# GalDude33/Fetal-MRI-Segmentation

Hardware: AMD Instinct MI355X
Metric: 3D patches/sec (64x128x128, bf16) fwd+bwd (higher is better)
Workload: dtype bf16

## Files before the change

### fetal-mri-segmentation_amd/csrc/conv3d_api.hip

```cpp
#include "common.h"

int conv3d_fwd_generic(const void*, int, int, int, const void*, int, const void*, const float*, const void*, void*, int, int, int, int, int,
                       int, float, int, hipStream_t);
int conv3d_wgrad_generic(const void*, int, int, int, const void*, int, const void*, float*, float*, int, int, int, int, int, int,
                         hipStream_t);
bool conv3d_fwd_mfma_ok(int C0, int C1, int Cout, int D, int H, int W, int dtype);
bool conv3d_wgrad_mfma_ok(int C0, int C1, int Cout, int D, int H, int W, int dtype);
bool conv3d_fwd_needs_cube(int D, int H, int W);
bool conv3d_wgrad_cout32_ok(int C0, int C1, int Cout, int N, int D, int H, int W, int dtype, int planar, int up0);
int conv3d_fwd_mfma(const void*, int, int, int, const void*, int, const void*, const float*, const void*, void*, int, int, int, int, int, int,
                    float, int, hipStream_t);
int conv3d_wgrad_mfma_f32(const void*, int, int, const void*, int, const void*, float*, float*, int, int, int, int, int, hipStream_t);
int conv3d_wgrad_mfma(const void*, int, int, int, const void*, int, const void*, float*, float*, int, int, int, int, int, void*, int64_t,
                      hipStream_t);
int64_t conv3d_wgrad_mfma_ws_bytes(int C0, int C1, int Cout, int N, int D, int H, int W, int planar);
int conv3d_upcat_wgrad_mfma(const void*, int, const void*, int, const void*, float*, float*, float*, int, int, int, int, int, int, void*, int64_t,
                            hipStream_t);
int conv3d_fwd_mfma_ex(int, const void*, int, int, int, const void*, int, const void*, const float*, const void*, const void*, void*, int, int, int,
                       int, int, int, float, int, hipStream_t);

int conv3d_upcat_wgrad_mfma_ex(const void*, int, const void*, int, const void*, float*, float*, float*, int, int, int, int, int, int, int, void*,
                               int64_t, hipStream_t);
int conv3d_fwd_mfma_res_b27(const void*, int, const void*, const float*, const void*, void*, int, int, int, int, int, int, float, int, hipStream_t);
int conv3d_fwd_tail_ok(int C0, int Cout, int N, int D, int H, int W, int dtype, int planar);
int conv3d_fwd_mfma_tail(const void*, int, const void*, const float*, void*, void*, const float*, const float*, float*, int, int, int, int, int, int,
                         float, int, int, hipStream_t);

int conv3d_fwd_ntail_ok(int C0, int C1, int Cout, int N, int D, int H, int W, int dtype);
int conv3d_fwd_mfma_ntail(int, const void*, int, int, const void*, int, const void*, const float*, const void*, void*, int, int, int, int, int, int,
                          float, double*, int, const float*, hipStream_t);
int norm_ws_zero(double* ws, int n, hipStream_t s);
int norm_ws_fold(double* ws, int nslot, int n, hipStream_t s);
int conv3d_fwd_ntail_slots();

bool conv3d_first_ok(int C0, int C1, int Cout, int D, int H, int W, int dtype, int up0, int planar);
int conv3d_first_fwd(const void*, int, int, const void*, const float*, void*, int, int, int, int, int, int, float, hipStream_t);
int conv3d_first_wgrad(const void*, int, int, const void*, float*, float*, int, int, int, int, int, hipStream_t);
bool conv3d_first_dgrad_ok(int Cin, int Cout, int D, int H, int W, int dtype);
int conv3d_first_dgrad(const void*, int, const void*, float*, int, int, int, int, int, hipStream_t);

static int check_common(const void* src0, int C0, int up0, int planar, const void* src1, int C1, int N, int D, int H, int W, int Cout) {
    if (N <= 0 || D <= 0 || H <= 0 || W <= 0 || Cout <= 0 || C0 <= 0 || C1 < 0) return FMRI_E_SHAPE;
    if (!src0 || (C1 > 0 && !src1)) return FMRI_E_SHAPE;
// ... 287 lines not shown
                if (!(cd == 1 && ch == 1 && cw == 1) && acc[ch][cw] != 0.f) atomicAdd(&out[((cd * 3 + ch) * 3 + cw) * C + c], acc[ch][cw]);
    }
}
}
extern "C" int fmri_conv3d_upcat_fwd_bias27(const void* src0_low, int C0, const void* src1, int C1, const void* w_up_fwd, const void* w_skip_fwd,
                                            const float* bias27, void* y, int N, int D, int H, int W, int Cout, int act, float alpha, int dtype,
                                            fmri_stream_t stream) {
    if (!src0_low || !src1 || !w_up_fwd || !w_skip_fwd || !bias27 || !y || N <= 0 || C1 <= 0) return FMRI_E_SHAPE;
    if (!(upcat_ok(C0, C1, Cout, D, H, W, dtype, 0) & 1)) return FMRI_E_SHAPE;
    if ((((uintptr_t)src0_low) | ((uintptr_t)src1) | ((uintptr_t)w_up_fwd) | ((uintptr_t)w_skip_fwd) | ((uintptr_t)y) | ((uintptr_t)bias27)) & 15) return FMRI_E_ALIGN;
    int rc = conv3d_fwd_mfma_ex(1, src0_low, C0, 0, 0, nullptr, 0, w_up_fwd, nullptr, nullptr, nullptr, y, N, D / 2, H / 2, W / 2, Cout, FMRI_ACT_NONE, 0.f,
                                dtype, as_stream(stream));
    if (rc) return rc;
    return conv3d_fwd_mfma_res_b27(src1, C1, w_skip_fwd, bias27, y, y, N, D, H, W, Cout, act, alpha, dtype, as_stream(stream));
}
extern "C" int fmri_conv3d_upcat_wgrad_parts(const void* src0_low, int C0, const void* src1, int C1, const void* dy, float* dw, float* db,
                                             float* dwc, int N, int D, int H, int W, int Cout, int dtype, void* workspace, int64_t workspace_bytes,
                                             fmri_stream_t stream) {
    if (!src0_low || !dy || !dw || !dwc || N <= 0 || C1 <= 0 || !src1) return FMRI_E_SHAPE;
    if (!(upcat_ok(C0, C1, Cout, D, H, W, dtype, 0) & 2)) return FMRI_E_SHAPE;
    if ((((uintptr_t)src0_low) | ((uintptr_t)src1) | ((uintptr_t)dy)) & 15) return FMRI_E_ALIGN;
    return conv3d_upcat_wgrad_mfma_ex(src0_low, C0, src1, C1, dy, dw, db, dwc, N, D, H, W, Cout, 0, 0, workspace, workspace_bytes, as_stream(stream));
}
extern "C" int fmri_border_class_sums(const void* dy, float* out27, int N, int D, int H, int W, int C, int dtype, fmri_stream_t stream) {
    if (!dy || !out27 || N <= 0 || D < 2 || H < 2 || W < 2 || C <= 0) return FMRI_E_SHAPE;
    hipStream_t s = as_stream(stream);
    const dim3 grid(N * D, H >= 64 ? 8 : (H >= 16 ? 4 : 1));
    if (dtype == FMRI_BF16) k_border_class_sums<bf16_t><<<grid, 256, 0, s>>>((const bf16_t*)dy, out27, D, H, W, C);
    else if (dtype == FMRI_F32) k_border_class_sums<float><<<grid, 256, 0, s>>>((const float*)dy, out27, D, H, W, C);
    else return FMRI_E_DTYPE;
    FMRI_LAUNCH_CHECK();
    return FMRI_OK;
}

extern "C" int64_t fmri_norm_tail_ws_doubles(int G, int C) { return (int64_t)(1 + conv3d_fwd_ntail_slots()) * G * C * 2; }
extern "C" int fmri_conv3d_fwd_ntail_ok(int C0, int C1, int Cout, int N, int D, int H, int W, int dtype) {
    if (N <= 0 || D <= 0 || H <= 0 || W <= 0 || C0 <= 0 || C1 < 0 || Cout <= 0) return 0;
    return conv3d_fwd_ntail_ok(C0, C1, Cout, N, D, H, W, dtype);
}
extern "C" int fmri_conv3d_fwd_stats(const void* src0, int C0, int up0, const void* src1, int C1, const void* w, const float* bias, void* y,
                                     int N, int D, int H, int W, int Cout, int act, float alpha, double* ws, int per_instance, int dtype,
                                     fmri_stream_t stream) {
    int rc = check_common(src0, C0, up0, 0, src1, C1, N, D, H, W, Cout);
    if (rc) return rc;
    if (!ws || !w || !y || !conv3d_fwd_ntail_ok(C0, C1, Cout, N, D, H, W, dtype)) return FMRI_E_SHAPE;
    if ((((uintptr_t)src0) | ((uintptr_t)src1) | ((uintptr_t)w) | ((uintptr_t)y) | ((uintptr_t)ws)) & 15) return FMRI_E_ALIGN;
// ... 85 lines not shown
```

### fetal-mri-segmentation_amd/csrc/conv3d_wgrad.hip

```cpp
#define FMRI_MFMA_TU_WGRAD
#include "mfma_common.h"

FMRI_DET_TU(mfma)

namespace {

namespace wg {
constexpr int TH = 8, TW = 16;
constexpr int XH = TH + 2, XW = TW + 2;
constexpr int XROWS = XH * XW;
constexpr int YROWS = TH * TW;
constexpr int NTHREADS = 256;
}


template <int ROWB> __device__ __forceinline__ int wg_slot_off(int row, int slot) {
    if (ROWB == 128) return row * 128 + ((slot ^ (((row >> 1) & 1) << 2)) << 4);
    return row * 64 + (slot << 4);
}

template <int ROWB>
__device__ __forceinline__ bf16x8_t tr_frag(const unsigned char* base, int row0, int tile32, int lane) {
    const int g = lane >> 4, q = (lane & 15) >> 2, p = lane & 3, hk = g >> 1;
    const int rowa = row0 + 8 * hk + q, rowb = rowa + 4;
// ... 567 lines not shown
__global__ void __launch_bounds__(256, F32 ? 1 : 2) k_conv_wgrad_kd(WkArgs a) {
    __shared__ __attribute__((aligned(16))) unsigned char lds[WkCfg<F32>::LDS_BYTES];
    const int lane = threadIdx.x & 63;
    const int wv = __builtin_amdgcn_readfirstlane(threadIdx.x >> 6);
    switch (wv & 3) {
        case 0: wk_run<0, F32>(a, lds, wv, lane); break;
        case 1: wk_run<1, F32>(a, lds, wv, lane); break;
        case 2: wk_run<2, F32>(a, lds, wv, lane); break;
        default: wk_run<3, F32>(a, lds, wv, lane); break;
    }
}

struct WuCfg {
    static constexpr int NW = 4;
    static constexpr int ROWB = 128, RS = 8;
    static constexpr int X_INSTR = (wg::XROWS * RS + 63) / 64;
    static constexpr int Y_INSTR = wg::YROWS * RS / 64;
    static constexpr int XS_BYTES = X_INSTR * 1024, YS_BYTES = Y_INSTR * 1024;
    static constexpr int NXS = 3, NYS = 2;
    static constexpr int LDS_BYTES = NXS * XS_BYTES + NYS * YS_BYTES;
    static constexpr int XPW = (X_INSTR + NW - 1) / NW, YPW = Y_INSTR / NW;
    static constexpr int PF = 3;
    static constexpr int SP0 = 1, SPD = 2;
};

template <int G>
__device__ __forceinline__ void wu_run(const WkArgs& a, unsigned char* lds, int wv, int lane) {
    typedef WuCfg K;
    constexpr int KDP = G >> 1, KHP = G & 1, NW = K::NW, ROWB = K::ROWB, RS = K::RS;
    constexpr int NI = 2;
    constexpr int XPW = K::XPW, YPW = K::YPW;
    typedef __attribute__((ext_vector_type(8))) short s16x8;
    const SrcB& s = a.s;
    const int N = a.N, D = a.D, H = a.H, W = a.W, Cout = a.Cout;
    const int Cin = s.C0;
    const int ncib = Cin / 64, ncob = Cout / 64;
    const int ncombo = 8 * ncob * ncib;
    const int wg_id = xcd_logical_id(blockIdx.x, gridDim.x);
    int combo = wg_id % ncombo;
    const int slab = wg_id / ncombo;
    const int cib = combo % ncib; combo /= ncib;
    const int cob = combo % ncob;
    const int par = combo / ncob;
    const int pd = par >> 2, ph = (par >> 1) & 1, pw = par & 1;
    const int co0 = cob * 64, cc = cib * 64;
    const int r = lane & 31, hk = lane >> 5;
    const bool do_bias = G == 0 && a.db != nullptr && cib == 0;

    f32x16 acc[2][2][NI];
#pragma unroll
    for (int q = 0; q < 4 * NI; ++q)
#pragma unroll
        for (int k = 0; k < 16; ++k) acc[q / (2 * NI)][(q / NI) & 1][q % NI][k] = 0.f;
    float bsum[2] = {0.f, 0.f};

    const int twn = W / wg::TW, thn = H / wg::TH;
    const int nunits = N * D * thn * twn;
    const unsigned lds0 = __builtin_amdgcn_readfirstlane(lds_addr(lds));

    int cn = 0, ch0 = 0, cw0 = 0;
    int x_off[XPW], y_off[YPW];
    unsigned x_ok = 0;
    auto col_setup = [&](int n, int h0, int w0) {
        cn = n; ch0 = h0; cw0 = w0;
        x_ok = 0;
#pragma unroll
        for (int k = 0; k < XPW; ++k) {
            const int id = wv + NW * k;
            const int i = id * 64 + lane;
            const int row = i / RS, ps = i % RS;
            const int ls = ps ^ (((row >> 1) & 1) << 2);
            const int xh = row / wg::XW, xw = row % wg::XW;
            const int gh = h0 - 1 + xh, gw = w0 - 1 + xw;
            const bool ok = id < K::X_INSTR && row < wg::XROWS && (unsigned)gh < (unsigned)H && (unsigned)gw < (unsigned)W;
            const int ghc = min(max(gh, 0), H - 1), gwc = min(max(gw, 0), W - 1);
            x_off[k] = ((ghc * W + gwc) * Cin + ls * 8) * 2;
// ... 1 lines not shown
        }
#pragma unroll
        for (int k = 0; k < YPW; ++k) {
            const int id = (NW - 1 - wv) + NW * k;
            const int i = id * 64 + lane;
            const int row = i / RS, ps = i % RS;
            const int ls = ps ^ (((row >> 1) & 1) << 2);
            y_off[k] = (((row >> 4) * 4 * W + (row & 15) * 2) * Cout + ls * 8) * 2;
        }
    };
    auto x_rsrc = [&](int gd) {
        const bool dok = (unsigned)gd < (unsigned)D;
        const int gdc = min(max(gd, 0), D - 1);
        return dma_rsrc(s.p0 + ((int64_t)cn * D + gdc) * H * W * Cin + cc, dok ? (int)DMA_OOB : 0);
    };
    auto y_rsrc = [&](int d) {
        return dma_rsrc(a.dy + ((((int64_t)cn * 2 * D + 2 * d + pd) * 2 * H + 2 * ch0 + ph) * 2 * W + 2 * cw0 + pw) * Cout + co0);
    };
    auto x_piece = [&](i32x4 rs, int slot, int k) {
        const int id = wv + NW * k;
        if (id < K::X_INSTR)
            dma16_buf(rs, ((x_ok >> k) & 1) ? (unsigned)x_off[k] : DMA_OOB, __builtin_amdgcn_readfirstlane(lds0 + slot * K::XS_BYTES + id * 1024));
    };
    auto y_piece = [&](i32x4 rs, int ybuf, int k) {
        const int id = (NW - 1 - wv) + NW * k;
        dma16_buf(rs, (unsigned)y_off[k], __builtin_amdgcn_readfirstlane(lds0 + K::NXS * K::XS_BYTES + ybuf * K::YS_BYTES + id * 1024));
    };
    auto issue_x = [&](int gd, int slot) {
        const i32x4 rs = x_rsrc(gd);
#pragma unroll
        for (int k = 0; k < XPW; ++k) x_piece(rs, slot, k);
    };
    auto issue_y = [&](int d, int ybuf) {
        const i32x4 rs = y_rsrc(d);
#pragma unroll
        for (int k = 0; k < YPW; ++k) y_piece(rs, ybuf, k);
    };

    const int gq = lane >> 4, qd = (lane & 15) >> 2, pp = lane & 3;
    const int lrow = 8 * (gq >> 1) + qd;
    const int lslot = 2 * (gq & 1) + (pp >> 1);
    const int shift = ph * wg::XW + pw;
    int pre_x[4];
#pragma unroll
    for (int m = 0; m < 4; ++m) pre_x[m] = wg_slot_off<ROWB>(lrow + shift + m, lslot) + (pp & 1) * 8;
    const int pre_y = wg_slot_off<ROWB>(lrow, lslot) + (pp & 1) * 8;

    const int per = (nunits + a.nslab - 1) / a.nslab;
    int u = slab * per;
    const int u_end = min(nunits, u + per);
    if (u < u_end) {
        int d;
        {
            int q = u;
            d = q % D; q /= D;
            const int w0 = (q % twn) * wg::TW; q /= twn;
            col_setup(q / thn, (q % thn) * wg::TH, w0);
        }
        issue_x(d + pd - 1, 0);
// ... 2 lines not shown
        int lo = 0, yb = 0;
#ifdef FMRI_PROF
        unsigned long long wprof[12] = {};
        PROF_T(wk0);
#endif
        for (; u < u_end; ++u) {
            PROF_T(w0);
            asm volatile("s_waitcnt vmcnt(0)" ::: "memory");
            PROF_T(w1);
            __builtin_amdgcn_s_barrier();
            PROF_T(w2);
            const bool more = u + 1 < u_end;
            const bool fresh = more && d + 1 == D;
            if (more && fresh) {
                int w0 = cw0 + wg::TW, h0 = ch0, n = cn;
                if (w0 == W) { w0 = 0; h0 += wg::TH; if (h0 == H) { h0 = 0; ++n; } }
                col_setup(n, h0, w0);
                d = -1;
            }
            PROF_T(w3);
            const int hi = lo == 2 ? 0 : lo + 1, fr = hi == 2 ? 0 : hi + 1;
            int xbase = (KDP ? hi : lo) * K::XS_BYTES;
            asm volatile("" : "+s"(xbase));
            const int ybase = K::NXS * K::XS_BYTES + yb * K::YS_BYTES;
            const int nyb = yb ^ 1;
            i32x4 nx_rs = {0, 0, 0, 0}, ny_rs = {0, 0, 0, 0};
            auto load_a = [&](int ks8, s16x8 (&av)[2]) {
#pragma unroll
                for (int h = 0; h < 2; ++h) {
                    const unsigned char* p0 = lds + ybase + (h ? (pre_y ^ 64) : pre_y) + ks8 * wg::TW * ROWB;
                    s16x4 v0 = __builtin_amdgcn_ds_read_tr16_b64_v4i16((lds_s16x4*)p0);
                    s16x4 v1 = __builtin_amdgcn_ds_read_tr16_b64_v4i16((lds_s16x4*)(p0 + 4 * ROWB));
                    av[h] = __builtin_shufflevector(v0, v1, 0, 1, 2, 3, 4, 5, 6, 7);
                }
            };
            auto load_b = [&](int st) {
                const int ks8 = st / (2 * NI), j = (st / NI) & 1, i = st % NI;
                const int c = (ks8 + KHP) * wg::XW + j;
                const unsigned char* pb = lds + xbase + (i ? (pre_x[c & 3] ^ 64) : pre_x[c & 3]) + (c >> 2) * 4 * ROWB;
                s16x4 v0 = __builtin_amdgcn_ds_read_tr16_b64_v4i16((lds_s16x4*)pb);
                s16x4 v1 = __builtin_amdgcn_ds_read_tr16_b64_v4i16((lds_s16x4*)(pb + 4 * ROWB));
                return __builtin_shufflevector(v0, v1, 0, 1, 2, 3, 4, 5, 6, 7);
            };
            constexpr int NS = 16 * NI, PF = K::PF, RING = PF + 1;
            s16x8 av[2][2], b[RING];
#pragma unroll
            for (int q = 0; q < PF; ++q) b[q] = load_b(q);
            load_a(0, av[0]);
#pragma unroll
            for (int st = 0; st < NS; ++st) {
                const int ks8 = st / (2 * NI), j = (st / NI) & 1, i = st % NI, ab = ks8 & 1;
                if (st + PF < NS) b[(st + PF) % RING] = load_b(st + PF);
                if (st % (2 * NI) == 1 && ks8 + 1 < 8) load_a(ks8 + 1, av[ab ^ 1]);
                if (st % (2 * NI) == 0 && do_bias) {
#pragma unroll
                    for (int h = 0; h < 2; ++h)
#pragma unroll
                        for (int q = 0; q < 8; ++q) bsum[h] += bf2f((unsigned short)av[ab][h][q]);
                }
                const bf16x8_t bb = __builtin_bit_cast(bf16x8_t, b[st % RING]);
#pragma unroll
                for (int h = 0; h < 2; ++h)
                    acc[j][h][i] = __builtin_amdgcn_mfma_f32_32x32x16_bf16(__builtin_bit_cast(bf16x8_t, av[ab][h]), bb, acc[j][h][i], 0, 0, 0);
                if (more) {
                    if (st == 0) {
                        nx_rs = x_rsrc(fresh ? pd - 1 : d + 1 + pd);
                        ny_rs = y_rsrc(d + 1);
                    }
                    if (st >= K::SP0 && (st - K::SP0) % K::SPD == 0 && (st - K::SP0) / K::SPD < XPW + YPW) {
                        const int pc = (st - K::SP0) / K::SPD;
                        if (pc < YPW) y_piece(ny_rs, nyb, pc);
                        else x_piece(nx_rs, fr, pc - YPW);
                    }
                }
                __builtin_amdgcn_sched_barrier(0);
            }
            asm volatile("s_waitcnt lgkmcnt(0)" ::: "memory");
            PROF_T(w4);
#ifdef FMRI_PROF
            wprof[0] += w1 - w0; wprof[1] += w2 - w1; wprof[2] += w3 - w2; wprof[3] += w4 - w3; wprof[6] += 1;
#endif
            if (fresh) {
                __builtin_amdgcn_s_barrier();
                issue_x(pd, lo);
                lo = fr;
            } else {
                lo = hi;
            }
            yb ^= 1;
            ++d;
#ifdef FMRI_PROF
            { PROF_T(w5); wprof[4] += w5 - w4; }
#endif
        }
#ifdef FMRI_PROF
        { PROF_T(wk1); wprof[5] = wk1 - wk0; }
        if (lane == 0) for (int i = 0; i < 7; ++i) atomicAdd(&g_prof[i], wprof[i]);
#endif
    }
#pragma unroll
    for (int j = 0; j < 2; ++j)
#pragma unroll
        for (int h = 0; h < 2; ++h)
#pragma unroll
            for (int i = 0; i < NI; ++i)
#pragma unroll
                for (int reg = 0; reg < 16; ++reg) {
                    const int co = co0 + h * 32 + (reg & 3) + 8 * (reg >> 2) + 4 * hk;
                    const int ci = cc + i * 32 + r;
                    atomicAdd(&a.dw[((int64_t)((par * 2 + KDP) * 4 + KHP * 2 + j) * Cout + co) * Cin + ci], acc[j][h][i][reg]);
                }
    if (do_bias) {
#pragma unroll
        for (int h = 0; h < 2; ++h) {
            float bq = bsum[h];
            bq += __shfl_down(bq, 32);
            if (hk == 0) atomicAdd(&a.db[co0 + h * 32 + r], bq);
        }
    }
}

__global__ void __launch_bounds__(256, 1) k_conv_wgrad_up_kd(WkArgs a) {
    __shared__ __attribute__((aligned(16))) unsigned char lds[WuCfg::LDS_BYTES];
    const int lane = threadIdx.x & 63;
    const int wv = __builtin_amdgcn_readfirstlane(threadIdx.x >> 6);
    switch (wv & 3) {
        case 0: wu_run<0>(a, lds, wv, lane); break;
        case 1: wu_run<1>(a, lds, wv, lane); break;
        case 2: wu_run<2>(a, lds, wv, lane); break;
        default: wu_run<3>(a, lds, wv, lane); break;
    }
}

template <int CIB>
__global__ void __launch_bounds__(256)
k_wgrad_reduce(const float* __restrict__ ws, float* __restrict__ dw, int Cout, int Cin, int nslab, int ncombo, int ncob, int ncib,
               int planar, int ksp) {
    constexpr int PER4 = 9 * 64 * CIB / 4;
    __shared__ float4 red[8][32];
    const int tx = threadIdx.x & 31, ty = threadIdx.x >> 5;
    const int64_t col = (int64_t)blockIdx.x * 32 + tx;
    const bool ok = col < (int64_t)ncombo * PER4;
    float4 a0 = make_float4(0.f, 0.f, 0.f, 0.f), a1 = a0, a2 = a0, a3 = a0;
    int combo = 0, e4 = 0;
    if (ok) {
        combo = (int)(col / PER4);
        e4 = (int)(col % PER4);
        const int nsl = nslab * ksp;
        const float4* base = reinterpret_cast<const float4*>(ws) + e4;
        int j = ty;
        for (; j + 24 < nsl; j += 32) {
            const int64_t i0 = ((int64_t)(j / ksp) * ncombo + combo) * ksp + (j % ksp);
            const int64_t i1 = ((int64_t)((j + 8) / ksp) * ncombo + combo) * ksp + ((j + 8) % ksp);
// ... 145 lines not shown
        const int64_t q = i / C0;
        const int co = (int)(q % Cout);
        const int t = (int)(q / Cout) + (planar ? 9 : 0);
        const int kd = t / 9, kh = (t / 3) % 3, kw = t % 3;
        float acc = 0.f;
        if (planar) {
#pragma unroll
            for (int p = 0; p < 4; ++p) {
                const int cls = tap_class_w(p >> 1, kh) * 2 + tap_class_w(p & 1, kw);
                acc += dwc[((int64_t)(p * 4 + cls) * Cout + co) * C0 + c0];
            }
        } else {
#pragma unroll
            for (int p = 0; p < 8; ++p) {
                const int cls = (tap_class_w(p >> 2, kd) * 2 + tap_class_w((p >> 1) & 1, kh)) * 2 + tap_class_w(p & 1, kw);
                acc += dwc[((int64_t)(p * 8 + cls) * Cout + co) * C0 + c0];
            }
        }
        dw[((int64_t)t * Cout + co) * dw_ld + c0] += acc;
    }
}
}

int conv3d_upcat_wgrad_mfma_ex(const void* src0_low, int C0, const void* src1, int C1, const void* dy, float* dw, float* db, float* dwc, int N,
                               int D, int H, int W, int Cout, int planar, int expand, void* workspace, int64_t workspace_bytes, hipStream_t st);
int conv3d_upcat_wgrad_mfma(const void* src0_low, int C0, const void* src1, int C1, const void* dy, float* dw, float* db, float* dwc, int N,
                            int D, int H, int W, int Cout, int planar, void* workspace, int64_t workspace_bytes, hipStream_t st) {
    return conv3d_upcat_wgrad_mfma_ex(src0_low, C0, src1, C1, dy, dw, db, dwc, N, D, H, W, Cout, planar, 1, workspace, workspace_bytes, st);
}
int conv3d_upcat_wgrad_mfma_ex(const void* src0_low, int C0, const void* src1, int C1, const void* dy, float* dw, float* db, float* dwc, int N,
                               int D, int H, int W, int Cout, int planar, int expand, void* workspace, int64_t workspace_bytes, hipStream_t st) {
    if (hipMemsetAsync(dwc, 0, (size_t)(planar ? 16 : 64) * Cout * C0 * sizeof(float), st) != hipSuccess) return FMRI_E_LAUNCH;
    {
        SrcB s{(const bf16_t*)src0_low, nullptr, C0, 0, 0, planar ? 0 : 1, planar};
        const int Dl = planar ? D : D / 2, Hl = H / 2, Wl = W / 2;
        const bool wide = C0 % 64 == 0;
        const int CIB = wide ? 64 : 32;
        const int combos = (planar ? 4 : 16) * (Cout / 64) * (C0 / CIB);
        const int nunits = N * Dl * (Hl / wg::TH) * (Wl / wg::TW);
        int nslab = (1536 + combos - 1) / combos;
        if (nslab > nunits) nslab = nunits;
        if (nslab < 1) nslab = 1;
        float* const dbu = C1 == 0 ? db : nullptr;
        static const int upw_kd = env_int("FMRI_UPW_KD", 1, {0, 1});
        if (upw_kd && !planar && wide && Cout % 64 == 0) {
            const int combos_kd = 8 * (Cout / 64) * (C0 / 64);
            int nsl = (fwd_cu_count() + combos_kd - 1) / combos_kd;
            if (nsl > nunits) nsl = nunits;
            if (nsl < 1) nsl = 1;
            const WkArgs wa{s, (const bf16_t*)dy, dwc, dbu, N, Dl, Hl, Wl, Cout, nsl, C0};
            k_conv_wgrad_up_kd<<<combos_kd * nsl, 256, 0, st>>>(wa);
        } else if (wide) k_conv_wgrad_mfma<2, true><<<combos * nslab, wg::NTHREADS, 0, st>>>(s, (const bf16_t*)dy, dwc, dbu, N, Dl, Hl, Wl, Cout, nslab, nullptr, C0);
        else k_conv_wgrad_mfma<1, true><<<combos * nslab, wg::NTHREADS, 0, st>>>(s, (const bf16_t*)dy, dwc, dbu, N, Dl, Hl, Wl, Cout, nslab, nullptr, C0);
    }
    if (expand) k_expand_up_wgrad<<<grid_for((int64_t)(planar ? 9 : 27) * Cout * C0, 256, 1024), 256, 0, st>>>(dwc, dw, Cout, C0, C0 + C1, planar);
    FMRI_LAUNCH_CHECK();
    if (C1 == 0) return FMRI_OK;
    return conv3d_wgrad_mfma_ld(src1, C1, 0, planar, nullptr, 0, dy, dw + C0, C0 + C1, db, N, D, H, W, Cout, workspace, workspace_bytes, st);
}
```

### fetal-mri-segmentation_amd/fmri_hip/_lib.py

```python
import ctypes as C
import os

F32, BF16 = 0, 1
F64 = 3
ACT_NONE, ACT_RELU, ACT_LEAKY = 0, 1, 2
IMPL_AUTO, IMPL_GENERIC, IMPL_MFMA = 0, 1, 2

_HERE = os.path.dirname(os.path.abspath(__file__))
LIB_PATH = os.environ.get("FMRI_LIB") or os.path.join(os.path.dirname(_HERE), "lib", "libfmri_hip.so")


class LibraryMissing(RuntimeError):
    pass


class FmriError(RuntimeError):
    pass


p, i32, i64, f32 = C.c_void_p, C.c_int, C.c_int64, C.c_float
u64, u32 = C.c_uint64, C.c_uint32

SIGNATURES = {
    "fmri_version": [],
# ... 82 lines not shown
    "fmri_rmsprop_step": [p, p, p, i64, f32, f32, f32, f32, p, f32, f32, p],
    "fmri_adam_step_ex": [p, p, p, p, p, i64, f32, f32, f32, f32, f32, p, f32, f32, p],
    "fmri_set_deterministic": [p, p, i64],
    "fmri_deterministic_finish": [p, p, i64, p],
    "fmri_set_deterministic_scratch": [p, i64],
    "fmri_norm_det_workspace_bytes": [i32, i64, i32, i32],
    "fmri_tile_gather": [p, i32, i32, i32, p, i32, i32, i32, i32, p, i32, p],
    "fmri_tile_gather_stack": [p, p, i32, i32, i32, p, i32, i32, i32, i32, i32, i32, p, i32, p],
    "fmri_tile_scatter_accumulate": [p, p, i32, i32, i32, i32, i32, p, p, i32, i32, i32, p],
    "fmri_tile_finalize": [p, p, p, p, i64, i32, p],
    "fmri_volume_pad_flip": [p, i32, i32, i32, i32, p, i32, i32, i32, i32, p, i32, C.c_double, p],
    "fmri_tile_finalize_flip": [p, p, i32, i32, i32, i32, p, i32, i32, i32, p, i32, p, p],
    "fmri_labels_expand_u8": [p, i64, p, i32, p, p],
    "fmri_tile_finalize_labels": [p, p, p, p, i64, i32, C.c_double, p, p],
    "fmri_cast": [p, i32, p, i32, i64, p],
    "fmri_conv3d_upcat_ok": [i32, i32, i32, i32, i32, i32, i32],
    "fmri_conv3d_upcat_fwd_bias27": [p, i32, p, i32, p, p, p, p, i32, i32, i32, i32, i32, i32, f32, i32, p],
    "fmri_conv3d_upcat_wgrad_parts": [p, i32, p, i32, p, p, p, p, i32, i32, i32, i32, i32, i32, p, i64, p],
    "fmri_border_class_sums": [p, p, i32, i32, i32, i32, i32, i32, p],
    "fmri_conv3d_pack_up_weights": [p, i32, i32, i32, p, p, p, p, i32, p],
    "fmri_conv3d_upcat_fwd": [p, i32, p, i32, p, p, p, p, i32, i32, i32, i32, i32, i32, f32, i32, p],
    "fmri_conv3d_upcat_dgrad": [p, i32, p, p, p, p, p, p, i32, i32, i32, i32, i32, i32, i32, p],
    "fmri_conv3d_stride2_fwd": [p, i32, p, p, p, i32, i32, i32, i32, i32, i32, p],
    "fmri_conv3d_upcat_wgrad": [p, i32, p, i32, p, p, p, p, i32, i32, i32, i32, i32, i32, p, i64, p],
    "fmri_conv2d_upcat_ok": [i32, i32, i32, i32, i32, i32, i32],
    "fmri_conv2d_pack_up_weights": [p, i32, i32, i32, p, p, p, p, i32, p],
    "fmri_conv2d_upcat_fwd": [p, i32, p, i32, p, p, p, p, i32, i32, i32, i32, i32, f32, i32, p],
    "fmri_conv2d_upcat_dgrad": [p, i32, p, p, p, p, p, p, i32, i32, i32, i32, i32, i32, p],
    "fmri_conv2d_upcat_wgrad": [p, i32, p, i32, p, p, p, p, i32, i32, i32, i32, i32, p, i64, p],
    "fmri_sigmoid_dice_fwd_weighted": [p, p, p, p, p, i64, p],
    "fmri_sigmoid_loss_bwd_weighted": [p, p, p, p, p, i64, i32, f32, f32, f32, p],
    "fmri_minmax": [p, i64, i32, p, p],
    "fmri_rescale_intensity": [p, i64, i32, p, i32, f32, f32, f32, p],
    "fmri_noise_augment": [p, i64, i32, p, p, i32, f32, p],
    "fmri_shot_noise_step": [p, i64, i32, p, p, p, p, i32, p],
    "fmri_correlate1d_f32": [p, p, i32, i32, i32, i32, p, i32, i32, p],
    "fmri_coarse_dropout": [p, i32, i32, i32, i32, i32, p, i32, i32, i32, p, p],
    "fmri_minmax_ws_batch": [p, i64, i64, i32, i32, p, p, p],
    "fmri_rescale_intensity_ws_batch": [p, i64, i64, i32, i32, p, p, p, p],
    "fmri_affine_sample_batch": [i32, p, p, p, p, i32, i32, p, p, i32, i32, i32, i32, i32, p, i32, i32, i64, p],
    "fmri_mri_intensity_ws_batch": [p, i32, i32, i32, i64, i32, i32, p, p, p, p, p],
    "fmri_noise_rng_batch": [p, i64, i64, i32, i32, p, p, i32, f32, u64, p, p],
    "fmri_shot_noise_rng_batch": [p, i64, i64, i32, i32, p, p, u64, p, p],
    "fmri_elastic_fields_rng_batch": [p, i32, i32, i32, p, p, u64, p, i32, p],
    "fmri_elastic_warp_batch": [p, i32, i32, i32, i32, i32, i64, p, i32, p, i32, i64, i32, p],
    "fmri_coarse_dropout_rng_batch": [p, i32, i32, i32, i32, i32, i64, i32, p, i32, f32, p, u64, p, p],
# ... 36 lines not shown
```

### fetal-mri-segmentation_amd/fmri_hip/ops.py

```python
import torch

from ._lib import lib, check, F32, BF16, F64, ACT_NONE, ACT_RELU, IMPL_AUTO


def dt(t):
    if t.dtype == torch.float32:
        return F32
    if t.dtype == torch.bfloat16:
        return BF16
    raise TypeError("unsupported dtype %s" % t.dtype)


import os as _os

_raw_stream = getattr(torch._C, "_cuda_getCurrentRawStream", None) if _os.environ.get("FMRI_RAW_STREAM", "1") != "0" else None
_cur_device = getattr(torch._C, "_cuda_getDevice", None)


def _s():
    if _raw_stream is not None and _cur_device is not None:
        return _raw_stream(_cur_device())
    return torch.cuda.current_stream().cuda_stream


# ... 695 lines not shown
    _need_cuda(x, w_s2_fwd, bias, y)
    N, D, H, W, Cin = x.shape
    Cout = y.shape[-1]
    assert tuple(y.shape) == (N, D // 2, H // 2, W // 2, Cout) and tuple(w_s2_fwd.shape) == (8, 8, Cout, Cin)
    assert bias is None or (bias.dtype == torch.float32 and bias.numel() >= Cout)
    check(lib().fmri_conv3d_stride2_fwd(_p(x), Cin, _p(w_s2_fwd), _p(bias), _p(y), N, D, H, W, Cout, dt(x), _s()), "fmri_conv3d_stride2_fwd")
    return y


def conv3d_upcat_wgrad(src0_low, src1, dy, dw, db, dwc_scratch, workspace=None, planar=False):
    _need_cuda(src0_low, src1, dy, dw, db, dwc_scratch, workspace)
    N, D, H, W, Cout = dy.shape
    C0, C1 = src0_low.shape[-1], (0 if src1 is None else src1.shape[-1])
    assert dwc_scratch.dtype == torch.float32 and dwc_scratch.numel() >= (16 if planar else 64) * Cout * C0
    nws = 0 if workspace is None else workspace.numel() * workspace.element_size()
    if planar:
        assert N == 1
        check(lib().fmri_conv2d_upcat_wgrad(_p(src0_low), C0, _p(src1), C1, _p(dy), _p(dw), _p(db), _p(dwc_scratch), D, H, W, Cout, dt(dy),
                                            _p(workspace), nws, _s()), "fmri_conv2d_upcat_wgrad")
        return
    check(lib().fmri_conv3d_upcat_wgrad(_p(src0_low), C0, _p(src1), C1, _p(dy), _p(dw), _p(db), _p(dwc_scratch), N, D, H, W, Cout, dt(dy),
                                        _p(workspace), nws, _s()),
          "fmri_conv3d_upcat_wgrad")


def conv3d_upcat_fwd_bias27(src0_low, src1, w_up_f, w_sk_f, bias27, y, act=ACT_RELU, alpha=0.0):
    _need_cuda(src0_low, src1, w_up_f, w_sk_f, bias27, y)
    N, D, H, W, Cout = y.shape
    assert bias27.dtype == torch.float32 and tuple(bias27.shape) == (27, Cout) and bias27.is_contiguous()
    check(lib().fmri_conv3d_upcat_fwd_bias27(_p(src0_low), src0_low.shape[-1], _p(src1), src1.shape[-1], _p(w_up_f), _p(w_sk_f), _p(bias27), _p(y),
                                             N, D, H, W, Cout, act, float(alpha), dt(y), _s()), "fmri_conv3d_upcat_fwd_bias27")
    return y


def conv3d_upcat_wgrad_parts(src0_low, src1, dy, dw, db, dwc, workspace=None):
    _need_cuda(src0_low, src1, dy, dw, db, dwc, workspace)
    N, D, H, W, Cout = dy.shape
    C0, C1 = src0_low.shape[-1], src1.shape[-1]
    assert dwc.dtype == torch.float32 and dwc.numel() >= 64 * Cout * C0 and tuple(dw.shape) == (27, Cout, C0 + C1)
    nws = 0 if workspace is None else workspace.numel() * workspace.element_size()
    check(lib().fmri_conv3d_upcat_wgrad_parts(_p(src0_low), C0, _p(src1), C1, _p(dy), _p(dw), _p(db), _p(dwc), N, D, H, W, Cout, dt(dy), _p(workspace),
                                              nws, _s()), "fmri_conv3d_upcat_wgrad_parts")


def border_class_sums(dy, out27):
    _need_cuda(dy, out27)
# ... 951 lines not shown
```

### include/fmri_hip.h

```cpp
#ifndef FMRI_HIP_H
#define FMRI_HIP_H
#include <stddef.h>
#include <stdint.h>

#ifdef __cplusplus
extern "C" {
#endif

typedef void* fmri_stream_t;

enum { FMRI_OK = 0, FMRI_E_SHAPE = -1, FMRI_E_ALIGN = -2, FMRI_E_ARCH = -3, FMRI_E_LAUNCH = -4, FMRI_E_DTYPE = -5 };
enum { FMRI_F32 = 0, FMRI_BF16 = 1, FMRI_U8 = 2 ,
       FMRI_F64 = 3  };
enum { FMRI_ACT_NONE = 0, FMRI_ACT_RELU = 1, FMRI_ACT_LEAKY = 2 };
enum { FMRI_IMPL_AUTO = 0, FMRI_IMPL_GENERIC = 1, FMRI_IMPL_MFMA = 2 };

int fmri_version(void);
const char* fmri_error_string(int code);
int fmri_clock_stamp(unsigned long long* out16, fmri_stream_t stream);
int fmri_conv3d_uses_mfma(int C0, int C1, int Cout, int D, int H, int W, int dtype);

int fmri_conv3d_fwd(const void* src0, int C0, int up0, const void* src1, int C1, const void* w, const float* bias,
                    const void* mask, void* y, int N, int D, int H, int W, int Cout, int act, float alpha, int dtype,
                    int impl, int planar, fmri_stream_t stream);
// ... 23 lines not shown
int fmri_conv3d_upcat_fwd_bias27(const void* src0_low, int C0, const void* src1, int C1, const void* w_up_fwd, const void* w_skip_fwd,
                                 const float* bias27, void* y, int N, int D, int H, int W, int Cout, int act, float alpha, int dtype,
                                 fmri_stream_t stream);
int fmri_conv3d_upcat_wgrad_parts(const void* src0_low, int C0, const void* src1, int C1, const void* dy, float* dw, float* db, float* dwc,
                                  int N, int D, int H, int W, int Cout, int dtype, void* workspace, int64_t workspace_bytes,
                                  fmri_stream_t stream);
int fmri_border_class_sums(const void* dy, float* out27, int N, int D, int H, int W, int C, int dtype, fmri_stream_t stream);

int fmri_conv3d_upcat_ok(int C0, int C1, int Cout, int D, int H, int W, int dtype);
int fmri_conv3d_pack_up_weights(const float* w, int C0, int C1, int Cout, void* w_up_fwd, void* w_up_dgrad, void* w_skip_fwd,
                                void* w_skip_dgrad, int dtype, fmri_stream_t stream);
int fmri_conv3d_upcat_fwd(const void* src0_low, int C0, const void* src1, int C1, const void* w_up_fwd, const void* w_skip_fwd,
                          const float* bias, void* y, int N, int D, int H, int W, int Cout, int act, float alpha, int dtype,
                          fmri_stream_t stream);
int fmri_conv3d_upcat_dgrad(const void* dy, int Cout, const void* w_up_dgrad, const void* w_skip_dgrad, const void* mask_low,
                            const void* mask_skip, void* dx_low, void* dx_skip, int N, int D, int H, int W, int C0, int C1, int dtype,
                            fmri_stream_t stream);
int fmri_conv3d_stride2_fwd(const void* x, int Cin, const void* w_s2_fwd, const float* bias, void* y, int N, int D, int H, int W, int Cout, int dtype,
                            fmri_stream_t stream);

int fmri_conv3d_upcat_wgrad(const void* src0_low, int C0, const void* src1, int C1, const void* dy, float* dw, float* db,
                            float* dwc_scratch, int N, int D, int H, int W, int Cout, int dtype, void* workspace, int64_t workspace_bytes,
                            fmri_stream_t stream);

int fmri_conv2d_upcat_ok(int C0, int C1, int Cout, int S, int H, int W, int dtype);
int fmri_conv2d_pack_up_weights(const float* w, int C0, int C1, int Cout, void* w_up_fwd, void* w_up_dgrad, void* w_skip_fwd,
                                void* w_skip_dgrad, int dtype, fmri_stream_t stream);
int fmri_conv2d_upcat_fwd(const void* src0_low, int C0, const void* src1, int C1, const void* w_up_fwd, const void* w_skip_fwd,
                          const float* bias, void* y, int S, int H, int W, int Cout, int act, float alpha, int dtype, fmri_stream_t stream);
int fmri_conv2d_upcat_dgrad(const void* dy, int Cout, const void* w_up_dgrad, const void* w_skip_dgrad, const void* mask_low,
                            const void* mask_skip, void* dx_low, void* dx_skip, int S, int H, int W, int C0, int C1, int dtype,
                            fmri_stream_t stream);
int fmri_conv2d_upcat_wgrad(const void* src0_low, int C0, const void* src1, int C1, const void* dy, float* dw, float* db,
                            float* dwc_scratch, int S, int H, int W, int Cout, int dtype, void* workspace, int64_t workspace_bytes,
                            fmri_stream_t stream);

int fmri_conv3d_pack_weights(const float* w, void* w_fwd, void* w_dgrad, int Cout, int Cin, int dtype,
                             fmri_stream_t stream);
int fmri_pack_weights_batched(const int64_t* table, int n_layers, int n_blocks, int dtype, fmri_stream_t stream);

int fmri_conv1x1_fwd(const void* x, const float* w, const float* b, float* logits, int64_t nvox, int C, int L,
                     int dtype, fmri_stream_t stream);
int fmri_conv1x1_bwd(const void* x, const float* w, const float* dlogits, void* dx, float* dw, float* db, int64_t nvox,
                     int C, int L, int relu_mask, int dtype, fmri_stream_t stream);

int fmri_sigmoid_dice_fwd(const float* logits, const uint8_t* y_true, float* probs, double* sums, int64_t n,
// ... 210 lines not shown
```

Before: 307.4.

## Pair adjacent W-parities per workgroup in upcat weight-gradient kernel to share x-tile loads

Adds a paired form of the transposed-conv (upcat) weight-gradient kernel where each workgroup handles two adjacent W-parities. It loads both dy slices but reuses one staged x tile across three shifted column taps. This halves the number of parity combos, and with it the redundant x DMA and LDS reads per workgroup. The cost is a larger LDS footprint, more accumulators per wave and a different DMA issue spacing. A heuristic picks the paired form by default when each slab has enough units, and the change also exposes a form-selection entry point for testing.

```diff
diff --git a/fetal-mri-segmentation_amd/csrc/conv3d_api.hip b/fetal-mri-segmentation_amd/csrc/conv3d_api.hip
--- a/fetal-mri-segmentation_amd/csrc/conv3d_api.hip
+++ b/fetal-mri-segmentation_amd/csrc/conv3d_api.hip
@@ -19,6 +19,8 @@
 int conv3d_fwd_mfma_ex(int, const void*, int, int, int, const void*, int, const void*, const float*, const void*, const void*, void*, int, int, int,
                        int, int, int, float, int, hipStream_t);
 
+int conv3d_upcat_wgrad_parity(int form, const void* src0_low, int C0, const void* dy, float* dwc, float* dbu, int N, int Dl, int Hl, int Wl, int Cout,
+                              int planar, hipStream_t st);
 int conv3d_upcat_wgrad_mfma_ex(const void*, int, const void*, int, const void*, float*, float*, float*, int, int, int, int, int, int, int, void*,
                                int64_t, hipStream_t);
 int conv3d_fwd_mfma_res_b27(const void*, int, const void*, const float*, const void*, void*, int, int, int, int, int, int, float, int, hipStream_t);
@@ -352,6 +354,17 @@
     if ((((uintptr_t)src0_low) | ((uintptr_t)src1) | ((uintptr_t)dy)) & 15) return FMRI_E_ALIGN;
     return conv3d_upcat_wgrad_mfma_ex(src0_low, C0, src1, C1, dy, dw, db, dwc, N, D, H, W, Cout, 0, 0, workspace, workspace_bytes, as_stream(stream));
 }
+extern "C" int fmri_conv3d_upcat_wgrad_form(int form, const void* src0_low, int C0, const void* dy, float* dwc, float* db, int N, int D, int H, int W,
+                                            int Cout, int planar, int dtype, fmri_stream_t stream) {
+    if (!src0_low || !dy || !dwc || N <= 0 || C0 <= 0 || Cout <= 0 || D <= 0 || H <= 0 || W <= 0) return FMRI_E_SHAPE;
+    if (dtype != FMRI_BF16) return FMRI_E_DTYPE;
+    if (((planar ? 0 : D) | H | W) & 1) return FMRI_E_SHAPE;
+    const int Dl = planar ? D : D / 2, Hl = H / 2, Wl = W / 2;
+    if (!conv3d_wgrad_mfma_ok(C0, 0, Cout, Dl, Hl, Wl, dtype)) return FMRI_E_SHAPE;
+    if ((long long)H * W * Cout * 2 >= (1ll << 31)) return FMRI_E_SHAPE;
+    if ((((uintptr_t)src0_low) | ((uintptr_t)dy)) & 15) return FMRI_E_ALIGN;
+    return conv3d_upcat_wgrad_parity(form, src0_low, C0, dy, dwc, db, N, Dl, Hl, Wl, Cout, planar ? 1 : 0, as_stream(stream));
+}
 extern "C" int fmri_border_class_sums(const void* dy, float* out27, int N, int D, int H, int W, int C, int dtype, fmri_stream_t stream) {
     if (!dy || !out27 || N <= 0 || D < 2 || H < 2 || W < 2 || C <= 0) return FMRI_E_SHAPE;
     hipStream_t s = as_stream(stream);
diff --git a/fetal-mri-segmentation_amd/csrc/conv3d_wgrad.hip b/fetal-mri-segmentation_amd/csrc/conv3d_wgrad.hip
--- a/fetal-mri-segmentation_amd/csrc/conv3d_wgrad.hip
+++ b/fetal-mri-segmentation_amd/csrc/conv3d_wgrad.hip
@@ -613,36 +613,40 @@
     static constexpr int XPW = (X_INSTR + NW - 1) / NW, YPW = Y_INSTR / NW;
     static constexpr int PF = 3;
     static constexpr int SP0 = 1, SPD = 2;
+    static constexpr int LDS_BYTES_P2 = NXS * XS_BYTES + 2 * NYS * YS_BYTES;
+    static constexpr int SPD_P2 = 3;
 };
 
-template <int G>
+template <int G, bool P2>
 __device__ __forceinline__ void wu_run(const WkArgs& a, unsigned char* lds, int wv, int lane) {
     typedef WuCfg K;
     constexpr int KDP = G >> 1, KHP = G & 1, NW = K::NW, ROWB = K::ROWB, RS = K::RS;
     constexpr int NI = 2;
+    constexpr int NPW = P2 ? 2 : 1;
     constexpr int XPW = K::XPW, YPW = K::YPW;
+    constexpr int YBASE = K::NXS * K::XS_BYTES;
     typedef __attribute__((ext_vector_type(8))) short s16x8;
     const SrcB& s = a.s;
     const int N = a.N, D = a.D, H = a.H, W = a.W, Cout = a.Cout;
     const int Cin = s.C0;
     const int ncib = Cin / 64, ncob = Cout / 64;
-    const int ncombo = 8 * ncob * ncib;
+    const int ncombo = (8 / NPW) * ncob * ncib;
     const int wg_id = xcd_logical_id(blockIdx.x, gridDim.x);
     int combo = wg_id % ncombo;
     const int slab = wg_id / ncombo;
     const int cib = combo % ncib; combo /= ncib;
     const int cob = combo % ncob;
-    const int par = combo / ncob;
+    const int par = (combo / ncob) * NPW;
     const int pd = par >> 2, ph = (par >> 1) & 1, pw = par & 1;
     const int co0 = cob * 64, cc = cib * 64;
     const int r = lane & 31, hk = lane >> 5;
     const bool do_bias = G == 0 && a.db != nullptr && cib == 0;
 
-    f32x16 acc[2][2][NI];
-#pragma unroll
-    for (int q = 0; q < 4 * NI; ++q)
-#pragma unroll
-        for (int k = 0; k < 16; ++k) acc[q / (2 * NI)][(q / NI) & 1][q % NI][k] = 0.f;
+    f32x16 acc[NPW][2][2][NI];
+#pragma unroll
+    for (int q = 0; q < NPW * 4 * NI; ++q)
+#pragma unroll
+        for (int k = 0; k < 16; ++k) acc[q / (4 * NI)][(q / (2 * NI)) & 1][(q / NI) & 1][q % NI][k] = 0.f;
     float bsum[2] = {0.f, 0.f};
 
     const int twn = W / wg::TW, thn = H / wg::TH;
@@ -690,9 +694,9 @@
         if (id < K::X_INSTR)
             dma16_buf(rs, ((x_ok >> k) & 1) ? (unsigned)x_off[k] : DMA_OOB, __builtin_amdgcn_readfirstlane(lds0 + slot * K::XS_BYTES + id * 1024));
     };
-    auto y_piece = [&](i32x4 rs, int ybuf, int k) {
+    auto y_piece = [&](i32x4 rs, int ybuf, int k, int c) {
         const int id = (NW - 1 - wv) + NW * k;
-        dma16_buf(rs, (unsigned)y_off[k], __builtin_amdgcn_readfirstlane(lds0 + K::NXS * K::XS_BYTES + ybuf * K::YS_BYTES + id * 1024));
+        dma16_buf(rs, (unsigned)(y_off[k] + c * Cout * 2), __builtin_amdgcn_readfirstlane(lds0 + YBASE + (NPW * ybuf + c) * K::YS_BYTES + id * 1024));
     };
     auto issue_x = [&](int gd, int slot) {
         const i32x4 rs = x_rsrc(gd);
@@ -702,7 +706,9 @@
     auto issue_y = [&](int d, int ybuf) {
         const i32x4 rs = y_rsrc(d);
 #pragma unroll
-        for (int k = 0; k < YPW; ++k) y_piece(rs, ybuf, k);
+        for (int c = 0; c < NPW; ++c)
+#pragma unroll
+            for (int k = 0; k < YPW; ++k) y_piece(rs, ybuf, k, c);
     };
 
     const int gq = lane >> 4, qd = (lane & 15) >> 2, pp = lane & 3;
@@ -751,59 +757,72 @@
             const int hi = lo == 2 ? 0 : lo + 1, fr = hi == 2 ? 0 : hi + 1;
             int xbase = (KDP ? hi : lo) * K::XS_BYTES;
             asm volatile("" : "+s"(xbase));
-            const int ybase = K::NXS * K::XS_BYTES + yb * K::YS_BYTES;
+            const int ybase = YBASE + NPW * yb * K::YS_BYTES;
             const int nyb = yb ^ 1;
             i32x4 nx_rs = {0, 0, 0, 0}, ny_rs = {0, 0, 0, 0};
-            auto load_a = [&](int ks8, s16x8 (&av)[2]) {
-#pragma unroll
-                for (int h = 0; h < 2; ++h) {
-                    const unsigned char* p0 = lds + ybase + (h ? (pre_y ^ 64) : pre_y) + ks8 * wg::TW * ROWB;
-                    s16x4 v0 = __builtin_amdgcn_ds_read_tr16_b64_v4i16((lds_s16x4*)p0);
-                    s16x4 v1 = __builtin_amdgcn_ds_read_tr16_b64_v4i16((lds_s16x4*)(p0 + 4 * ROWB));
-                    av[h] = __builtin_shufflevector(v0, v1, 0, 1, 2, 3, 4, 5, 6, 7);
-                }
+            constexpr int NSH = NPW + 1, SPK = NSH * NI;
+            auto load_a = [&](int ks8, s16x8 (&av)[NPW][2]) {
+#pragma unroll
+                for (int c = 0; c < NPW; ++c)
+#pragma unroll
+                    for (int h = 0; h < 2; ++h) {
+                        const unsigned char* p0 = lds + ybase + c * K::YS_BYTES + (h ? (pre_y ^ 64) : pre_y) + ks8 * wg::TW * ROWB;
+                        s16x4 v0 = __builtin_amdgcn_ds_read_tr16_b64_v4i16((lds_s16x4*)p0);
+                        s16x4 v1 = __builtin_amdgcn_ds_read_tr16_b64_v4i16((lds_s16x4*)(p0 + 4 * ROWB));
+                        av[c][h] = __builtin_shufflevector(v0, v1, 0, 1, 2, 3, 4, 5, 6, 7);
+                    }
             };
             auto load_b = [&](int st) {
-                const int ks8 = st / (2 * NI), j = (st / NI) & 1, i = st % NI;
+                const int ks8 = st / SPK, j = (st / NI) % NSH, i = st % NI;
                 const int c = (ks8 + KHP) * wg::XW + j;
                 const unsigned char* pb = lds + xbase + (i ? (pre_x[c & 3] ^ 64) : pre_x[c & 3]) + (c >> 2) * 4 * ROWB;
                 s16x4 v0 = __builtin_amdgcn_ds_read_tr16_b64_v4i16((lds_s16x4*)pb);
                 s16x4 v1 = __builtin_amdgcn_ds_read_tr16_b64_v4i16((lds_s16x4*)(pb + 4 * ROWB));
                 return __builtin_shufflevector(v0, v1, 0, 1, 2, 3, 4, 5, 6, 7);
             };
-            constexpr int NS = 16 * NI, PF = K::PF, RING = PF + 1;
-            s16x8 av[2][2], b[RING];
+            constexpr int NS = 8 * SPK, PF = K::PF, RING = PF + 1;
+            constexpr int SPD = P2 ? K::SPD_P2 : K::SPD, NYP = NPW * YPW;
+            static_assert(K::SP0 + SPD * (XPW + NYP - 1) < NS, "every DMA piece of the next unit needs a step of this one");
+            s16x8 av[2][NPW][2], b[RING];
 #pragma unroll
             for (int q = 0; q < PF; ++q) b[q] = load_b(q);
             load_a(0, av[0]);
-#pragma unroll
-            for (int st = 0; st < NS; ++st) {
-                const int ks8 = st / (2 * NI), j = (st / NI) & 1, i = st % NI, ab = ks8 & 1;
+            static_for<NS>([&](auto st_tag) {
+                constexpr int st = decltype(st_tag)::value;
+                constexpr int ks8 = st / SPK, j = (st / NI) % NSH, i = st % NI, ab = ks8 & 1;
                 if (st + PF < NS) b[(st + PF) % RING] = load_b(st + PF);
-                if (st % (2 * NI) == 1 && ks8 + 1 < 8) load_a(ks8 + 1, av[ab ^ 1]);
-                if (st % (2 * NI) == 0 && do_bias) {
-#pragma unroll
-                    for (int h = 0; h < 2; ++h)
-#pragma unroll
-                        for (int q = 0; q < 8; ++q) bsum[h] += bf2f((unsigned short)av[ab][h][q]);
+                if (st % SPK == NPW && ks8 + 1 < 8) load_a(ks8 + 1, av[ab ^ 1]);
+                if (st % SPK == 0 && do_bias) {
+#pragma unroll
+                    for (int c = 0; c < NPW; ++c)
+#pragma unroll
+                        for (int h = 0; h < 2; ++h)
+#pragma unroll
+                            for (int q = 0; q < 8; ++q) bsum[h] += bf2f((unsigned short)av[ab][c][h][q]);
                 }
                 const bf16x8_t bb = __builtin_bit_cast(bf16x8_t, b[st % RING]);
 #pragma unroll
-                for (int h = 0; h < 2; ++h)
-                    acc[j][h][i] = __builtin_amdgcn_mfma_f32_32x32x16_bf16(__builtin_bit_cast(bf16x8_t, av[ab][h]), bb, acc[j][h][i], 0, 0, 0);
+                for (int c = 0; c < NPW; ++c) {
+                    const int kw = j - c;
+                    if (kw >= 0 && kw <= 1) {
+#pragma unroll
+                        for (int h = 0; h < 2; ++h)
+                            acc[c][kw][h][i] = __builtin_amdgcn_mfma_f32_32x32x16_bf16(__builtin_bit_cast(bf16x8_t, av[ab][c][h]), bb, acc[c][kw][h][i], 0, 0, 0);
+                    }
+                }
                 if (more) {
                     if (st == 0) {
                         nx_rs = x_rsrc(fresh ? pd - 1 : d + 1 + pd);
                         ny_rs = y_rsrc(d + 1);
                     }
-                    if (st >= K::SP0 && (st - K::SP0) % K::SPD == 0 && (st - K::SP0) / K::SPD < XPW + YPW) {
-                        const int pc = (st - K::SP0) / K::SPD;
-                        if (pc < YPW) y_piece(ny_rs, nyb, pc);
-                        else x_piece(nx_rs, fr, pc - YPW);
+                    if constexpr (st >= K::SP0 && (st - K::SP0) % SPD == 0 && (st - K::SP0) / SPD < XPW + NYP) {
+                        constexpr int pc = (st - K::SP0) / SPD;
+                        if constexpr (pc < NYP) y_piece(ny_rs, nyb, pc % YPW, pc / YPW);
+                        else x_piece(nx_rs, fr, pc - NYP);
                     }
                 }
                 __builtin_amdgcn_sched_barrier(0);
-            }
+            });
             asm volatile("s_waitcnt lgkmcnt(0)" ::: "memory");
             PROF_T(w4);
 #ifdef FMRI_PROF
@@ -828,17 +847,19 @@
 #endif
     }
 #pragma unroll
-    for (int j = 0; j < 2; ++j)
-#pragma unroll
-        for (int h = 0; h < 2; ++h)
-#pragma unroll
-            for (int i = 0; i < NI; ++i)
-#pragma unroll
-                for (int reg = 0; reg < 16; ++reg) {
-                    const int co = co0 + h * 32 + (reg & 3) + 8 * (reg >> 2) + 4 * hk;
-                    const int ci = cc + i * 32 + r;
-                    atomicAdd(&a.dw[((int64_t)((par * 2 + KDP) * 4 + KHP * 2 + j) * Cout + co) * Cin + ci], acc[j][h][i][reg]);
-                }
+    for (int c = 0; c < NPW; ++c)
+#pragma unroll
+        for (int j = 0; j < 2; ++j)
+#pragma unroll
+            for (int h = 0; h < 2; ++h)
+#pragma unroll
+                for (int i = 0; i < NI; ++i)
+#pragma unroll
+                    for (int reg = 0; reg < 16; ++reg) {
+                        const int co = co0 + h * 32 + (reg & 3) + 8 * (reg >> 2) + 4 * hk;
+                        const int ci = cc + i * 32 + r;
+                        atomicAdd(&a.dw[((int64_t)(((par + c) * 2 + KDP) * 4 + KHP * 2 + j) * Cout + co) * Cin + ci], acc[c][j][h][i][reg]);
+                    }
     if (do_bias) {
 #pragma unroll
         for (int h = 0; h < 2; ++h) {
@@ -849,15 +870,16 @@
     }
 }
 
+template <bool P2>
 __global__ void __launch_bounds__(256, 1) k_conv_wgrad_up_kd(WkArgs a) {
-    __shared__ __attribute__((aligned(16))) unsigned char lds[WuCfg::LDS_BYTES];
+    __shared__ __attribute__((aligned(16))) unsigned char lds[P2 ? WuCfg::LDS_BYTES_P2 : WuCfg::LDS_BYTES];
     const int lane = threadIdx.x & 63;
     const int wv = __builtin_amdgcn_readfirstlane(threadIdx.x >> 6);
     switch (wv & 3) {
-        case 0: wu_run<0>(a, lds, wv, lane); break;
-        case 1: wu_run<1>(a, lds, wv, lane); break;
-        case 2: wu_run<2>(a, lds, wv, lane); break;
-        default: wu_run<3>(a, lds, wv, lane); break;
+        case 0: wu_run<0, P2>(a, lds, wv, lane); break;
+        case 1: wu_run<1, P2>(a, lds, wv, lane); break;
+        case 2: wu_run<2, P2>(a, lds, wv, lane); break;
+        default: wu_run<3, P2>(a, lds, wv, lane); break;
     }
 }
 
@@ -1049,36 +1071,60 @@
 }
 }
 
+enum { UPW_PER_KD = 0, UPW_KD_SHARING = 1, UPW_PAIRED = 2 };
 int conv3d_upcat_wgrad_mfma_ex(const void* src0_low, int C0, const void* src1, int C1, const void* dy, float* dw, float* db, float* dwc, int N,
                                int D, int H, int W, int Cout, int planar, int expand, void* workspace, int64_t workspace_bytes, hipStream_t st);
 int conv3d_upcat_wgrad_mfma(const void* src0_low, int C0, const void* src1, int C1, const void* dy, float* dw, float* db, float* dwc, int N,
                             int D, int H, int W, int Cout, int planar, void* workspace, int64_t workspace_bytes, hipStream_t st) {
     return conv3d_upcat_wgrad_mfma_ex(src0_low, C0, src1, C1, dy, dw, db, dwc, N, D, H, W, Cout, planar, 1, workspace, workspace_bytes, st);
 }
-int conv3d_upcat_wgrad_mfma_ex(const void* src0_low, int C0, const void* src1, int C1, const void* dy, float* dw, float* db, float* dwc, int N,
-                               int D, int H, int W, int Cout, int planar, int expand, void* workspace, int64_t workspace_bytes, hipStream_t st) {
+int conv3d_upcat_wgrad_parity(int form, const void* src0_low, int C0, const void* dy, float* dwc, float* dbu, int N, int Dl, int Hl, int Wl, int Cout,
+                              int planar, hipStream_t st) {
+    const bool wide = C0 % 64 == 0;
+    if (form < UPW_PER_KD || form > UPW_PAIRED || (form != UPW_PER_KD && (planar || !wide || Cout % 64))) return FMRI_E_SHAPE;
     if (hipMemsetAsync(dwc, 0, (size_t)(planar ? 16 : 64) * Cout * C0 * sizeof(float), st) != hipSuccess) return FMRI_E_LAUNCH;
-    {
-        SrcB s{(const bf16_t*)src0_low, nullptr, C0, 0, 0, planar ? 0 : 1, planar};
-        const int Dl = planar ? D : D / 2, Hl = H / 2, Wl = W / 2;
-        const bool wide = C0 % 64 == 0;
+    SrcB s{(const bf16_t*)src0_low, nullptr, C0, 0, 0, planar ? 0 : 1, planar};
+    const int nunits = N * Dl * (Hl / wg::TH) * (Wl / wg::TW);
+    if (form == UPW_PER_KD) {
         const int CIB = wide ? 64 : 32;
         const int combos = (planar ? 4 : 16) * (Cout / 64) * (C0 / CIB);
-        const int nunits = N * Dl * (Hl / wg::TH) * (Wl / wg::TW);
         int nslab = (1536 + combos - 1) / combos;
         if (nslab > nunits) nslab = nunits;
         if (nslab < 1) nslab = 1;
+        if (wide) k_conv_wgrad_mfma<2, true><<<combos * nslab, wg::NTHREADS, 0, st>>>(s, (const bf16_t*)dy, dwc, dbu, N, Dl, Hl, Wl, Cout, nslab, nullptr, C0);
+        else k_conv_wgrad_mfma<1, true><<<combos * nslab, wg::NTHREADS, 0, st>>>(s, (const bf16_t*)dy, dwc, dbu, N, Dl, Hl, Wl, Cout, nslab, nullptr, C0);
+    } else {
+        const int combos_kd = (form == UPW_PAIRED ? 4 : 8) * (Cout / 64) * (C0 / 64);
+        int nsl = (fwd_cu_count() + combos_kd - 1) / combos_kd;
+        if (nsl > nunits) nsl = nunits;
+        if (nsl < 1) nsl = 1;
+        const WkArgs wa{s, (const bf16_t*)dy, dwc, dbu, N, Dl, Hl, Wl, Cout, nsl, C0};
+        if (form == UPW_PAIRED) k_conv_wgrad_up_kd<true><<<combos_kd * nsl, 256, 0, st>>>(wa);
+        else k_conv_wgrad_up_kd<false><<<combos_kd * nsl, 256, 0, st>>>(wa);
+    }
+    FMRI_LAUNCH_CHECK();
+    return FMRI_OK;
+}
+constexpr int UPW_PAIR_MIN_UNITS = 128;
+static int upcat_wgrad_form(int C0, int Cout, int N, int Dl, int Hl, int Wl, int planar) {
+    static const int upw_kd = env_int("FMRI_UPW_KD", 2, {0, 1, 2});
+    if (!upw_kd || planar || (C0 % 64) || (Cout % 64)) return UPW_PER_KD;
+    if (upw_kd == 2) {
+        const int combos2 = 4 * (Cout / 64) * (C0 / 64);
+        const int nunits = N * Dl * (Hl / wg::TH) * (Wl / wg::TW);
+        int nsl = (fwd_cu_count() + combos2 - 1) / combos2;
+        if (nsl > nunits) nsl = nunits;
+        if (nunits / nsl >= UPW_PAIR_MIN_UNITS) return UPW_PAIRED;
+    }
+    return UPW_KD_SHARING;
+}
+int conv3d_upcat_wgrad_mfma_ex(const void* src0_low, int C0, const void* src1, int C1, const void* dy, float* dw, float* db, float* dwc, int N,
+                               int D, int H, int W, int Cout, int planar, int expand, void* workspace, int64_t workspace_bytes, hipStream_t st) {
+    {
+        const int Dl = planar ? D : D / 2, Hl = H / 2, Wl = W / 2;
         float* const dbu = C1 == 0 ? db : nullptr;
-        static const int upw_kd = env_int("FMRI_UPW_KD", 1, {0, 1});
-        if (upw_kd && !planar && wide && Cout % 64 == 0) {
-            const int combos_kd = 8 * (Cout / 64) * (C0 / 64);
-            int nsl = (fwd_cu_count() + combos_kd - 1) / combos_kd;
-            if (nsl > nunits) nsl = nunits;
-            if (nsl < 1) nsl = 1;
-            const WkArgs wa{s, (const bf16_t*)dy, dwc, dbu, N, Dl, Hl, Wl, Cout, nsl, C0};
-            k_conv_wgrad_up_kd<<<combos_kd * nsl, 256, 0, st>>>(wa);
-        } else if (wide) k_conv_wgrad_mfma<2, true><<<combos * nslab, wg::NTHREADS, 0, st>>>(s, (const bf16_t*)dy, dwc, dbu, N, Dl, Hl, Wl, Cout, nslab, nullptr, C0);
-        else k_conv_wgrad_mfma<1, true><<<combos * nslab, wg::NTHREADS, 0, st>>>(s, (const bf16_t*)dy, dwc, dbu, N, Dl, Hl, Wl, Cout, nslab, nullptr, C0);
+        const int rc = conv3d_upcat_wgrad_parity(upcat_wgrad_form(C0, Cout, N, Dl, Hl, Wl, planar), src0_low, C0, dy, dwc, dbu, N, Dl, Hl, Wl, Cout, planar, st);
+        if (rc != FMRI_OK) return rc;
     }
     if (expand) k_expand_up_wgrad<<<grid_for((int64_t)(planar ? 9 : 27) * Cout * C0, 256, 1024), 256, 0, st>>>(dwc, dw, Cout, C0, C0 + C1, planar);
     FMRI_LAUNCH_CHECK();
diff --git a/fetal-mri-segmentation_amd/fmri_hip/_lib.py b/fetal-mri-segmentation_amd/fmri_hip/_lib.py
--- a/fetal-mri-segmentation_amd/fmri_hip/_lib.py
+++ b/fetal-mri-segmentation_amd/fmri_hip/_lib.py
@@ -128,6 +128,7 @@
     "fmri_conv3d_upcat_fwd": [p, i32, p, i32, p, p, p, p, i32, i32, i32, i32, i32, i32, f32, i32, p],
     "fmri_conv3d_upcat_dgrad": [p, i32, p, p, p, p, p, p, i32, i32, i32, i32, i32, i32, i32, p],
     "fmri_conv3d_stride2_fwd": [p, i32, p, p, p, i32, i32, i32, i32, i32, i32, p],
+    "fmri_conv3d_upcat_wgrad_form": [i32, p, i32, p, p, p, i32, i32, i32, i32, i32, i32, i32, p],
     "fmri_conv3d_upcat_wgrad": [p, i32, p, i32, p, p, p, p, i32, i32, i32, i32, i32, i32, p, i64, p],
     "fmri_conv2d_upcat_ok": [i32, i32, i32, i32, i32, i32, i32],
     "fmri_conv2d_pack_up_weights": [p, i32, i32, i32, p, p, p, p, i32, p],
diff --git a/fetal-mri-segmentation_amd/fmri_hip/ops.py b/fetal-mri-segmentation_amd/fmri_hip/ops.py
--- a/fetal-mri-segmentation_amd/fmri_hip/ops.py
+++ b/fetal-mri-segmentation_amd/fmri_hip/ops.py
@@ -741,6 +741,20 @@
     check(lib().fmri_conv3d_upcat_wgrad(_p(src0_low), C0, _p(src1), C1, _p(dy), _p(dw), _p(db), _p(dwc_scratch), N, D, H, W, Cout, dt(dy),
                                         _p(workspace), nws, _s()),
           "fmri_conv3d_upcat_wgrad")
+
+
+UPW_FORM_PER_KD, UPW_FORM_KD_SHARING, UPW_FORM_PAIRED = 0, 1, 2
+
+
+def conv3d_upcat_wgrad_form(form, src0_low, dy, dwc, db=None, planar=False):
+    _need_cuda(src0_low, dy, dwc, db)
+    N, D, H, W, Cout = dy.shape
+    C0 = src0_low.shape[-1]
+    assert dwc.dtype == torch.float32 and dwc.numel() >= (16 if planar else 64) * Cout * C0
+    assert db is None or (db.dtype == torch.float32 and db.numel() >= Cout)
+    assert tuple(src0_low.shape[:-1]) == ((N, D, H // 2, W // 2) if planar else (N, D // 2, H // 2, W // 2))
+    check(lib().fmri_conv3d_upcat_wgrad_form(int(form), _p(src0_low), C0, _p(dy), _p(dwc), _p(db), N, D, H, W, Cout, 1 if planar else 0, dt(dy), _s()),
+          "fmri_conv3d_upcat_wgrad_form")
 
 
 def conv3d_upcat_fwd_bias27(src0_low, src1, w_up_f, w_sk_f, bias27, y, act=ACT_RELU, alpha=0.0):
diff --git a/include/fmri_hip.h b/include/fmri_hip.h
--- a/include/fmri_hip.h
+++ b/include/fmri_hip.h
@@ -69,6 +69,12 @@
 int fmri_conv3d_upcat_wgrad(const void* src0_low, int C0, const void* src1, int C1, const void* dy, float* dw, float* db,
                             float* dwc_scratch, int N, int D, int H, int W, int Cout, int dtype, void* workspace, int64_t workspace_bytes,
                             fmri_stream_t stream);
+
+#define FMRI_UPW_FORM_PER_KD 0
+#define FMRI_UPW_FORM_KD_SHARING 1
+#define FMRI_UPW_FORM_PAIRED 2
+int fmri_conv3d_upcat_wgrad_form(int form, const void* src0_low, int C0, const void* dy, float* dwc, float* db, int N, int D, int H, int W,
+                                 int Cout, int planar, int dtype, fmri_stream_t stream);
 
 int fmri_conv2d_upcat_ok(int C0, int C1, int Cout, int S, int H, int W, int dtype);
 int fmri_conv2d_pack_up_weights(const float* w, int C0, int C1, int Cout, void* w_up_fwd, void* w_up_dgrad, void* w_skip_fwd,
```

Result: no change. 307.8, median of 6 (+0.1%).
